# gabrieldemarmiesse/mojo-simdjson

Measured on AMD Instinct MI355X. Metric: stage-1 GB/s JSON ingested (+ % HBM3E peak), 1/2/4/8 MI355X, higher is better.
Workload: dtype u8

## Files before the change

### include/msj_stage1.h

```cpp
#ifndef MSJ_STAGE1_H
#define MSJ_STAGE1_H

#include <stdint.h>

#ifdef __cplusplus
extern "C" {
#endif

#define MSJ_SUCCESS 0
#define MSJ_CAPACITY 1
#define MSJ_MEMALLOC 2
#define MSJ_UTF8_ERROR 11
#define MSJ_EMPTY 13
#define MSJ_UNESCAPED_CHARS 14
#define MSJ_UNCLOSED_STRING 15
#define MSJ_UNEXPECTED_ERROR 24
#define MSJ_ERR_BAD_ARGUMENT (-1)
#define MSJ_ERR_NO_DEVICE (-2)
#define MSJ_ERR_HIP (-3)

#define MSJ_FLAG_STRICT_UTF8 1u
#define MSJ_FLAG_NO_UTF8 2u
#define MSJ_FLAG_TWO_PASS 0x100u
#define MSJ_FLAG_DEBUG_STALL 0x200u
// ... 112 lines not shown
int32_t msj_sharded_create(msj_ctx *ctx, const msj_exchange *xchg, const msj_sharded_ops *ops, msj_sharded **out);
void msj_sharded_destroy(msj_sharded *sh);
uint64_t msj_sharded_reruns(const msj_sharded *sh);
uint64_t msj_sharded_rounds(const msj_sharded *sh);
typedef struct msj_sharded_stats {
    uint64_t results, rounds, reruns;
    uint64_t stitch_device_ns, result_wait_ns;
    uint64_t kernel_device_ns;
    uint64_t last_kernel_ns;
    uint64_t last_stitch_ns;
    uint64_t reruns_behind_queue;
    uint64_t reserved[3];
} msj_sharded_stats;
int32_t msj_sharded_get_stats(const msj_sharded *sh, msj_sharded_stats *out);
#define MSJ_SHARDED_KERNEL_DONE 1
#define MSJ_SHARDED_REPORTS_IN 2
int32_t msj_sharded_ticket_state(msj_sharded *sh, uint32_t ticket);
void msj_exchange_release(msj_exchange *x);

int32_t msj_stage1_sharded_submit(msj_sharded *sh, const uint8_t *d_shard, uint64_t shard_len, uint32_t *d_idx,
                                  uint64_t idx_capacity, uint64_t total_len, int32_t has_prefix,
                                  const msj_carry *speculation, msj_segment *d_segments, uint32_t max_segments,
                                  void *stream, uint32_t flags, uint32_t *ticket_out);
typedef struct msj_shard_placement {
    uint64_t index_begin;
    uint64_t byte_base;
    uint64_t count;
    uint64_t bytes;
} msj_shard_placement;
int32_t msj_stage1_sharded_result(msj_sharded *sh, uint32_t ticket, int32_t *code_out, uint64_t *total_count_out,
                                  msj_carry *local_out, msj_carry *used_out, msj_shard_placement *placement_out);
int32_t msj_debug_set_pipeline_min_bytes(msj_ctx *ctx, uint64_t bytes);
int32_t msj_debug_fail_pipeline_setup(msj_ctx *ctx, int32_t on);
int32_t msj_debug_set_segment_bytes(msj_ctx *ctx, uint64_t bytes);

typedef struct msj_tokens_result {
    uint64_t n;
    int32_t final_depth;
    int32_t min_depth;
    int32_t max_depth;
    uint32_t reserved;
} msj_tokens_result;

int32_t msj_tokens_device(msj_ctx *ctx, const uint8_t *d_buf, uint64_t len, const uint32_t *d_idx, uint64_t n,
                          uint8_t *d_type, int32_t *d_depth, uint32_t *d_match, msj_tokens_result *d_result,
                          void *stream);
int32_t msj_tokens_chain_device(msj_ctx *ctx, const uint8_t *d_buf, uint64_t len, const uint32_t *d_idx, uint64_t n,
                                uint8_t *d_type, int32_t *d_depth, uint32_t *d_match, msj_tokens_result *d_result,
                                const msj_tokens_result *d_prev, void *stream);

#define MSJ_SPAN_STRING 1u
#define MSJ_SPAN_ESCAPED 2u
#define MSJ_SPAN_NUMBER 4u
#define MSJ_SPAN_FLOAT 8u
#define MSJ_SPAN_OPEN 16u
#define MSJ_SPAN_BAD 32u
#define MSJ_SPAN_LONG 128u
int32_t msj_token_spans_device(msj_ctx *ctx, const uint8_t *d_buf, uint64_t len, const uint32_t *d_idx, uint64_t n,
                               uint32_t *d_end, uint8_t *d_flags, void *stream);

typedef struct msj_bracket_pair {
    uint32_t open, close;
} msj_bracket_pair;
int32_t msj_tokens_pairs_device(msj_ctx *ctx, const uint8_t *d_buf, uint64_t len, const uint32_t *d_idx, uint64_t n, uint8_t *d_type,
                                int32_t *d_depth, msj_bracket_pair *d_pairs, msj_tokens_result *d_result,
                                const msj_tokens_result *d_prev, void *stream);
// ... 269 lines not shown
```

### mojo_simdjson_amd/csrc/ctx.h

```cpp
#pragma once
#include <hip/hip_runtime.h>

#include <mutex>
#include <vector>

#include "../../include/msj_stage1.h"
#include "launch.h"
#include "stage1_kernel.h"

#pragma GCC visibility push(hidden)

inline bool hip_ok(hipError_t e) { return e == hipSuccess; }
inline bool aligned(const void *p, uintptr_t a) { return (reinterpret_cast<uintptr_t>(p) & (a - 1)) == 0; }

struct DeviceBuffer {
    void *p = nullptr;
    uint64_t bytes = 0;
    DeviceBuffer() = default;
    DeviceBuffer(const DeviceBuffer &) = delete;
    DeviceBuffer &operator=(const DeviceBuffer &) = delete;
    ~DeviceBuffer() { release(); }
    bool reserve(uint64_t need, bool headroom) {
        if (need <= bytes) return true;
        release();
// ... 8 lines not shown
    void release() {
        if (p) {
            (void)hipDeviceSynchronize();
            (void)hipFree(p);
        }
        p = nullptr;
        bytes = 0;
    }
    template <class T>
    T *as() const { return static_cast<T *>(p); }
};

constexpr uint64_t kPipelineMinDefault = 64u << 20;

struct HostPipe;

struct msj_ctx {
    int device = 0;
    HostPipe *pipe = nullptr;
    DeviceBuffer ws;
    uint64_t ws_words = 0;
    uint32_t ws_toggle = 0;
    uint32_t ws_dirty[2] = {0, 0};
    msj_carry *carries = nullptr;
    uint32_t n_carries = 0;
    DeviceBuffer d_in, d_idx;
    msj_carry *d_result = nullptr;
    uint8_t *h_pin = nullptr;
    uint8_t *d_small = nullptr;
    uint32_t grid = 0;
    uint32_t wait_ticks = msj::kWaitTicksDefault;
    uint64_t seg_bytes = msj::kSegmentBytes;
    uint64_t pipeline_min = kPipelineMinDefault;
    bool pipe_unavailable = false;
    bool pipe_fail_setup = false;
    DeviceBuffer tp;
    uint64_t fallbacks = 0;
    struct {
        bool valid = false;
        const uint8_t *d_buf; uint64_t len; uint32_t *d_idx; uint64_t idx_capacity;
        const msj_carry *d_carry_in; msj_carry *d_carry_out; msj_segment *d_segments; uint32_t max_segments;
        bool has_prefix, is_final, no_emit; uint64_t trailer_len; hipStream_t stream; uint32_t flags;
        bool by_value; uint32_t carry_bits;
    } last;
    struct HostRange { const uint8_t *base; uint64_t bytes; };
    std::vector<HostRange> pinned;
    bool is_pinned(const void *p, uint64_t n) const {
        const uint8_t *q = static_cast<const uint8_t *>(p);
        for (const HostRange &r : pinned)
            if (q >= r.base && n <= r.bytes && (uint64_t)(q - r.base) <= r.bytes - n) return true;
        return false;
    }
    DeviceBuffer span_fix;
    DeviceBuffer tok_ws;
    uint64_t tok_doc_n = ~0ull;
    DeviceBuffer seg_idx;
    uint8_t *types_out = nullptr;
    DeviceBuffer resid;
    msj_token_opts tok_opts;
    DeviceBuffer doc_ws;
    DeviceBuffer num_ws;
    DeviceBuffer val_ws;
    DeviceBuffer vdoc_ws;
    DeviceBuffer tape_ws;
    DeviceBuffer tdoc_ws;
    DeviceBuffer sel_ws;
// ... 22 lines not shown
```

### mojo_simdjson_amd/csrc/host_pipe.cpp

```cpp
#include <atomic>
#include <chrono>
#include <condition_variable>
#include <cstdio>
#include <cstdlib>
#include <cstring>
#include <deque>
#include <functional>
#include <new>
#include <thread>

#include <pthread.h>
#include <sched.h>
#include <sys/syscall.h>
#include <unistd.h>

#include "ctx.h"

#pragma GCC visibility push(hidden)

struct GpuHostLocality {
    char pci[32] = "";
    int node = -1;
    cpu_set_t cpus;
    int n_cpus = 0;
    char link_speed[32] = "", link_width[16] = "";
};
static bool read_line(const char *path, char *out, size_t cap) {
    FILE *f = std::fopen(path, "r");
    if (!f) return false;
    const bool ok = std::fgets(out, (int)cap, f) != nullptr;
    std::fclose(f);
    if (ok) out[std::strcspn(out, "\n")] = 0;
    return ok;
}
static GpuHostLocality gpu_locality(int device) {
    GpuHostLocality g;
    CPU_ZERO(&g.cpus);
    char bus[32] = "";
    if (hipDeviceGetPCIBusId(bus, (int)sizeof bus, device) != hipSuccess) {
        (void)hipGetLastError();
        return g;
    }
    for (char *c = bus; *c; c++)
        if (*c >= 'A' && *c <= 'F') *c = (char)(*c - 'A' + 'a');
    std::snprintf(g.pci, sizeof g.pci, "%s", bus);
    char path[128], line[4096];
    std::snprintf(path, sizeof path, "/sys/bus/pci/devices/%s/numa_node", bus);
    if (read_line(path, line, sizeof line)) g.node = std::atoi(line);
    std::snprintf(path, sizeof path, "/sys/bus/pci/devices/%s/current_link_speed", bus);
    (void)read_line(path, g.link_speed, sizeof g.link_speed);
    std::snprintf(path, sizeof path, "/sys/bus/pci/devices/%s/current_link_width", bus);
    (void)read_line(path, g.link_width, sizeof g.link_width);
    std::snprintf(path, sizeof path, "/sys/bus/pci/devices/%s/local_cpulist", bus);
    cpu_set_t allowed;
    CPU_ZERO(&allowed);
    if (read_line(path, line, sizeof line) && sched_getaffinity(0, sizeof allowed, &allowed) == 0) {
        char *save = nullptr;
        for (char *tok = strtok_r(line, ",", &save); tok; tok = strtok_r(nullptr, ",", &save)) {
            int lo = 0, hi = 0;
            const int k = std::sscanf(tok, "%d-%d", &lo, &hi);
            if (k == 1) hi = lo;
            for (int c = lo; k >= 1 && c <= hi && c < CPU_SETSIZE; c++)
                if (CPU_ISSET(c, &allowed)) {
                    CPU_SET(c, &g.cpus);
                    g.n_cpus++;
                }
        }
    }
    return g;
}
static int numa_node_of(const void *p) {
#ifdef SYS_get_mempolicy
    int node = -1;
    if (p && syscall(SYS_get_mempolicy, &node, nullptr, 0UL, const_cast<void *>(p), 3UL ) == 0) return node;
#endif
    (void)p;
    return -1;
}

struct CopyPool {
    const cpu_set_t *bind = nullptr;
    int bound = 0;
    std::vector<std::thread> threads;
    std::deque<std::function<void()>> tasks;
    std::mutex m;
    std::condition_variable cv;
    bool stop = false;
    explicit CopyPool(int n, const cpu_set_t *cpus = nullptr) : bind(cpus) {
        std::atomic<int> ok{0};
        for (int i = 0; i < n; i++)
            threads.emplace_back([this, &ok] {
                if (bind && pthread_setaffinity_np(pthread_self(), sizeof(cpu_set_t), bind) == 0) ok.fetch_add(1);
                ok.fetch_add(1 << 16);
                for (;;) {
                    std::function<void()> f;
                    {
                        std::unique_lock<std::mutex> lk(m);
                        cv.wait(lk, [this] { return stop || !tasks.empty(); });
                        if (stop && tasks.empty()) return;
                        f = std::move(tasks.front());
                        tasks.pop_front();
                    }
                    f();
                }
            });
        while ((ok.load() >> 16) < n) std::this_thread::yield();
        bound = ok.load() & 0xFFFF;
    }
    ~CopyPool() {
        {
            std::lock_guard<std::mutex> lk(m);
            stop = true;
        }
        cv.notify_all();
        for (auto &t : threads) t.join();
    }
    void copy_async(void *dst, const void *src, uint64_t n, int parts, std::atomic<int> *pending) {
        if (parts < 1) parts = 1;
        pending->store(parts, std::memory_order_relaxed);
        const uint64_t step = ((n / parts) + 63) & ~63ull;
        for (int i = 0; i < parts; i++) {
            const uint64_t lo = step * i < n ? step * i : n, hi = (i + 1 == parts || step * (i + 1) > n) ? n : step * (i + 1);
            {
                std::lock_guard<std::mutex> lk(m);
                tasks.emplace_back([=] {
                    if (hi > lo) std::memcpy(static_cast<char *>(dst) + lo, static_cast<const char *>(src) + lo, hi - lo);
                    pending->fetch_sub(1, std::memory_order_release);
                });
            }
            cv.notify_one();
        }
    }
    static void wait(std::atomic<int> *pending) {
        while (pending->load(std::memory_order_acquire) != 0) std::this_thread::yield();
    }
    void copy(void *dst, const void *src, uint64_t n, int parts) {
        if (n < (1u << 20) || parts <= 1) {
            std::memcpy(dst, src, n);
            return;
        }
        std::mutex dm;
        std::condition_variable dcv;
        int left = parts;
        const uint64_t step = ((n / parts) + 63) & ~63ull;
        for (int i = 0; i < parts; i++) {
            const uint64_t lo = step * i < n ? step * i : n, hi = (i + 1 == parts || step * (i + 1) > n) ? n : step * (i + 1);
            {
                std::lock_guard<std::mutex> lk(m);
                tasks.emplace_back([=, &dm, &dcv, &left] {
                    if (hi > lo) std::memcpy(static_cast<char *>(dst) + lo, static_cast<const char *>(src) + lo, hi - lo);
                    std::lock_guard<std::mutex> g(dm);
                    if (--left == 0) dcv.notify_one();
                });
            }
            cv.notify_one();
        }
        std::unique_lock<std::mutex> lk(dm);
        dcv.wait(lk, [&] { return left == 0; });
    }
};

#ifdef MSJ_DEBUG_KNOBS
static int knob_int(const char *name, int dflt, int lo) {
    const char *v = std::getenv(name);
    const int x = v && *v ? std::atoi(v) : dflt;
    return x < lo ? lo : x;
}
bool knob_set(const char *name) { return std::getenv(name) != nullptr; }
#else
static int knob_int(const char *, int dflt, int) { return dflt; }
bool knob_set(const char *) { return false; }
#endif

struct HostPipe {
    static constexpr int kInSlots = 3, kOutSlots = 2;
    const int kCopyThreads = knob_int("MSJ_PIPE_THREADS", 8, 1), kParts = knob_int("MSJ_PIPE_PARTS", 4, 1);
    const bool direct_upload = knob_int("MSJ_PIPE_DIRECT_UPLOAD", 0, 0) != 0;
    static constexpr uint64_t kChunk = 16ull << 20;
    static constexpr uint64_t kPiece = 16ull << 20;
    uint8_t *pin_in[kInSlots] = {nullptr, nullptr, nullptr};
    uint8_t *pin_out[kOutSlots] = {nullptr, nullptr};
    msj_carry *h_carries = nullptr;
    msj_carry *d_carries = nullptr;
    uint64_t n_carries = 0;
    hipStream_t s_up = nullptr, s_k = nullptr, s_down = nullptr;
    hipEvent_t ev_in[kInSlots] = {nullptr, nullptr, nullptr};
    hipEvent_t ev_out[kOutSlots] = {nullptr, nullptr};
    std::vector<hipEvent_t> ev_chunk;
    GpuHostLocality where;
    CopyPool pool;
    bool ok = false;

    explicit HostPipe(int device) : where(gpu_locality(device)), pool(kCopyThreads, where.n_cpus > 0 ? &where.cpus : nullptr) {
        ok = true;
        std::thread([&] {
            (void)hipSetDevice(device);
            if (where.n_cpus > 0) (void)pthread_setaffinity_np(pthread_self(), sizeof(cpu_set_t), &where.cpus);
            for (auto &p : pin_in) {
                ok = ok && hip_ok(hipHostMalloc(reinterpret_cast<void **>(&p), kChunk, hipHostMallocDefault));
                if (ok) std::memset(p, 0, kChunk);
            }
            for (auto &p : pin_out) {
                ok = ok && hip_ok(hipHostMalloc(reinterpret_cast<void **>(&p), kPiece, hipHostMallocDefault));
                if (ok) std::memset(p, 0, kPiece);
            }
        }).join();
        ok = ok && hip_ok(hipStreamCreateWithFlags(&s_up, hipStreamNonBlocking)) &&
             hip_ok(hipStreamCreateWithFlags(&s_k, hipStreamNonBlocking)) &&
             hip_ok(hipStreamCreateWithFlags(&s_down, hipStreamNonBlocking));
        for (auto &e : ev_in) ok = ok && hip_ok(hipEventCreateWithFlags(&e, hipEventDisableTiming));
        for (auto &e : ev_out) ok = ok && hip_ok(hipEventCreateWithFlags(&e, hipEventDisableTiming));
    }
    ~HostPipe() {
        for (auto p : pin_in)
            if (p) (void)hipHostFree(p);
        for (auto p : pin_out)
            if (p) (void)hipHostFree(p);
        if (h_carries) (void)hipHostFree(h_carries);
        if (d_carries) (void)hipFree(d_carries);
        for (auto e : ev_in)
            if (e) (void)hipEventDestroy(e);
        for (auto e : ev_out)
            if (e) (void)hipEventDestroy(e);
        for (auto e : ev_chunk) (void)hipEventDestroy(e);
        if (s_up) (void)hipStreamDestroy(s_up);
        if (s_k) (void)hipStreamDestroy(s_k);
        if (s_down) (void)hipStreamDestroy(s_down);
    }
    bool reserve(uint64_t nchunks) {
        if (nchunks + 1 > n_carries) {
            if (h_carries) (void)hipHostFree(h_carries);
            if (d_carries) (void)hipFree(d_carries);
            h_carries = nullptr;
            d_carries = nullptr;
            n_carries = 0;
            if (!hip_ok(hipHostMalloc(reinterpret_cast<void **>(&h_carries), (nchunks + 1) * sizeof(msj_carry), hipHostMallocDefault)) ||
                !hip_ok(hipMalloc(reinterpret_cast<void **>(&d_carries), (nchunks + 1) * sizeof(msj_carry))))
                return false;
            n_carries = nchunks + 1;
        }
        while (ev_chunk.size() < nchunks) {
            hipEvent_t e;
            if (!hip_ok(hipEventCreateWithFlags(&e, hipEventDisableTiming))) return false;
            ev_chunk.push_back(e);
        }
        return true;
    }
};

void host_pipe_destroy(HostPipe *pipe) { delete pipe; }

int32_t host_pipeline(msj_ctx *ctx, const uint8_t *buf, uint64_t len, uint32_t *idx_out, uint64_t dev_cap, uint32_t flags,
                      msj_carry *res) {
    if (ctx->pipe_fail_setup) return kPipeUnavailable;
    if (!ctx->pipe) {
        ctx->pipe = new (std::nothrow) HostPipe(ctx->device);
        if (!ctx->pipe) return kPipeUnavailable;
    }
    HostPipe &P = *ctx->pipe;
    if (!P.ok) return kPipeUnavailable;
    uint8_t *const d_in = ctx->d_in.as<uint8_t>();
    uint32_t *const d_idx = ctx->d_idx.as<uint32_t>();
    const uint64_t chunk = HostPipe::kChunk;
    const uint64_t nchunks = (len + chunk - 1) / chunk;
    if (!P.reserve(nchunks)) return kPipeUnavailable;
    if (!hip_ok(hipMemsetAsync(&P.d_carries[0], 0, sizeof(msj_carry), P.s_k))) return kPipeUnavailable;

    static const bool trace = knob_set("MSJ_PIPE_TRACE");
    auto now = [] { return std::chrono::duration<double, std::milli>(std::chrono::steady_clock::now().time_since_epoch()).count(); };
    const double t_begin = now();
    std::vector<double> t_chunk_done(nchunks, 0.0), t_piece;
    const bool in_pinned = P.direct_upload || ctx->is_pinned(buf, len);
    const bool out_pinned = ctx->is_pinned(idx_out, dev_cap * sizeof(uint32_t));
    int32_t down_rc = MSJ_SUCCESS;
    std::atomic<bool> abort{false};
    std::atomic<uint64_t> recorded{0};
    std::thread down([&] {
        (void)hipSetDevice(ctx->device);
        uint64_t sent = 0, pieces = 0;
        std::atomic<int> copying[HostPipe::kOutSlots];
        for (auto &c : copying) c.store(0);
        for (uint64_t k = 0; k < nchunks; k++) {
            while (recorded.load(std::memory_order_acquire) <= k && !abort.load()) std::this_thread::yield();
            if (abort.load()) break;
            if (!hip_ok(hipEventSynchronize(P.ev_chunk[k]))) { down_rc = MSJ_ERR_HIP; break; }
            if (abort.load()) break;
            if (trace) t_chunk_done[k] = now() - t_begin;
            const msj_carry &c = P.h_carries[k + 1];
            const bool last = k + 1 == nchunks;
            uint64_t avail = c.count;
            if (last && (c.code == MSJ_SUCCESS || c.code == MSJ_EMPTY || c.code == MSJ_UTF8_ERROR)) avail += 3;
            if (avail > dev_cap) avail = dev_cap;
            if (out_pinned) {
                if (avail > sent &&
                    !hip_ok(hipMemcpyAsync(idx_out + sent, d_idx + sent, (avail - sent) * sizeof(uint32_t), hipMemcpyDeviceToHost, P.s_down))) {
                    down_rc = MSJ_ERR_HIP;
                    break;
                }
                sent = avail;
                if (trace) t_piece.push_back(now() - t_begin);
                continue;
            }
            const uint64_t piece = HostPipe::kPiece / sizeof(uint32_t);
            while (sent < avail) {
                const uint64_t mis = sent & 63u;
                const uint64_t n = avail - sent < piece - mis ? avail - sent : piece - mis;
                const int slot = (int)(pieces % HostPipe::kOutSlots);
                CopyPool::wait(&copying[slot]);
                if (!hip_ok(hipMemcpyAsync(P.pin_out[slot], d_idx + (sent - mis), (n + mis) * sizeof(uint32_t), hipMemcpyDeviceToHost, P.s_down)) ||
                    !hip_ok(hipStreamSynchronize(P.s_down))) {
                    down_rc = MSJ_ERR_HIP;
                    break;
                }
                P.pool.copy_async(idx_out + sent, P.pin_out[slot] + mis * sizeof(uint32_t), n * sizeof(uint32_t), P.kParts, &copying[slot]);
                sent += n;
                pieces++;
                if (trace) t_piece.push_back(now() - t_begin);
            }
            if (down_rc != MSJ_SUCCESS) break;
        }
        for (auto &c : copying) CopyPool::wait(&c);
        if (out_pinned && !hip_ok(hipStreamSynchronize(P.s_down))) down_rc = MSJ_ERR_HIP;
    });

    double t_copy = 0, t_wait = 0;
    int32_t rc = MSJ_SUCCESS;
    for (uint64_t k = 0; k < nchunks && rc == MSJ_SUCCESS; k++) {
        const uint64_t off = k * chunk, n = len - off < chunk ? len - off : chunk;
        const int slot = (int)(k % HostPipe::kInSlots);
        double t0 = now();
        if (in_pinned) {
            if (!hip_ok(hipMemcpyAsync(d_in + off, buf + off, n, hipMemcpyHostToDevice, P.s_up))) rc = MSJ_ERR_HIP;
            t_copy += now() - t0;
        } else {
            if (k >= (uint64_t)HostPipe::kInSlots && !hip_ok(hipEventSynchronize(P.ev_in[slot]))) rc = MSJ_ERR_HIP;
            double t1 = now();
            if (rc == MSJ_SUCCESS) P.pool.copy(P.pin_in[slot], buf + off, n, P.kParts);
            t_wait += t1 - t0;
            t_copy += now() - t1;
            if (rc == MSJ_SUCCESS && !hip_ok(hipMemcpyAsync(d_in + off, P.pin_in[slot], n, hipMemcpyHostToDevice, P.s_up)))
                rc = MSJ_ERR_HIP;
        }
        if (rc == MSJ_SUCCESS && (!hip_ok(hipEventRecord(P.ev_in[slot], P.s_up)) || !hip_ok(hipStreamWaitEvent(P.s_k, P.ev_in[slot], 0))))
            rc = MSJ_ERR_HIP;
        if (rc == MSJ_SUCCESS)
            rc = enqueue_shard(ctx, d_in + off, n, d_idx, dev_cap, &P.d_carries[k], &P.d_carries[k + 1], nullptr, 0, nullptr,
                               k > 0, k + 1 == nchunks, false, len, P.s_k, flags, (uint32_t)off);
        if (rc == MSJ_SUCCESS &&
            (!hip_ok(hipMemcpyAsync(&P.h_carries[k + 1], &P.d_carries[k + 1], sizeof(msj_carry), hipMemcpyDeviceToHost, P.s_k)) ||
             !hip_ok(hipEventRecord(P.ev_chunk[k], P.s_k))))
            rc = MSJ_ERR_HIP;
        if (rc == MSJ_SUCCESS) recorded.store(k + 1, std::memory_order_release);
        if (rc != MSJ_SUCCESS) {
            abort.store(true);
            for (uint64_t j = k; j < nchunks; j++) (void)hipEventRecord(P.ev_chunk[j], P.s_k);
        }
    }
    const double t_up = now();
    down.join();
    (void)hipStreamSynchronize(P.s_k);
    if (trace)
        std::fprintf(stderr, "msj host pipeline: %llu chunks, upload loop %.2f ms (slot waits %.2f, staging copies %.2f), "
                             "then %.2f ms until the last index was down\n",
                     (unsigned long long)nchunks, t_up - t_begin, t_wait, t_copy, now() - t_up);
    if (trace) {
        std::fprintf(stderr, "  chunk results seen at (ms):");
        for (double t : t_chunk_done) std::fprintf(stderr, " %.2f", t);
        std::fprintf(stderr, "\n  download pieces issued+previous copied out at (ms):");
        for (double t : t_piece) std::fprintf(stderr, " %.2f", t);
        std::fprintf(stderr, "\n");
    }
    ctx->last.valid = false;
    if (rc != MSJ_SUCCESS) return rc;
    if (down_rc != MSJ_SUCCESS) return down_rc;
    *res = P.h_carries[nchunks];
    return MSJ_SUCCESS;
}
#pragma GCC visibility pop

extern "C" {

int32_t msj_host_placement(msj_ctx *ctx, char *out, uint64_t capacity) {
    if (!out || capacity == 0) return MSJ_ERR_BAD_ARGUMENT;
    std::unique_lock<std::mutex> lock(g_default_mutex, std::defer_lock);
    if (!ctx) {
        lock.lock();
        ctx = default_ctx_locked();
        if (!ctx) return MSJ_ERR_NO_DEVICE;
    }
    const GpuHostLocality g = ctx->pipe ? ctx->pipe->where : gpu_locality(ctx->device);
    const int ring_in = ctx->pipe ? numa_node_of(ctx->pipe->pin_in[0]) : -1, ring_out = ctx->pipe ? numa_node_of(ctx->pipe->pin_out[0]) : -1;
    int nodes = 0;
    for (;; nodes++) {
        char path[64];
        std::snprintf(path, sizeof path, "/sys/devices/system/node/node%d", nodes);
        if (access(path, F_OK) != 0) break;
    }
    const int n = std::snprintf(out, (size_t)capacity,
                                "{\"gpu_pci\": \"%s\", \"gpu_numa_node\": %d, \"numa_nodes\": %d, \"gpu_local_cpus_usable\": %d, "
                                "\"pipeline_created\": %s, \"copy_threads\": %d, \"copy_threads_bound_to_gpu_node\": %d, "
                                "\"ring_in_node\": %d, \"ring_out_node\": %d, \"pcie_link_speed\": \"%s\", \"pcie_link_width\": \"%s\"}",
                                g.pci, g.node, nodes, g.n_cpus, ctx->pipe ? "true" : "false", ctx->pipe ? ctx->pipe->kCopyThreads : 0,
                                ctx->pipe ? ctx->pipe->pool.bound : 0, ring_in, ring_out, g.link_speed, g.link_width);
    return (n < 0 || (uint64_t)n >= capacity) ? MSJ_CAPACITY : MSJ_SUCCESS;
}

int32_t msj_debug_numa_node_of(const void *host_ptr) { return numa_node_of(host_ptr); }

}
```

Measured before the change: 3441.

## Restructure host pipeline into slot-ring issuer/drainer with L3-spread copy workers

Replaces the host staging pipeline with explicit input/output slot rings (4 in, 3 out by default instead of 3/2), a templated issuer and drainer state machine, a persistent parked drainer thread, and a lock-light ring-based copy pool whose workers are spread across L3 cache domains of the GPU-local CPUs. Chunks come from a schedule helper that can cap the chunk size. The aim is to overlap host staging copies, H2D uploads, kernels and D2H downloads more deeply, and to cut per-call thread creation and std::function queue overhead. In exchange it adds more pinned memory, more complex synchronisation, and affinity choices that depend on sysfs topology.

```diff
diff --git a/include/msj_stage1.h b/include/msj_stage1.h
--- a/include/msj_stage1.h
+++ b/include/msj_stage1.h
@@ -168,6 +168,7 @@
                                   msj_carry *local_out, msj_carry *used_out, msj_shard_placement *placement_out);
 int32_t msj_debug_set_pipeline_min_bytes(msj_ctx *ctx, uint64_t bytes);
 int32_t msj_debug_fail_pipeline_setup(msj_ctx *ctx, int32_t on);
+int32_t msj_debug_set_pipeline_chunk_bytes(msj_ctx *ctx, uint64_t bytes);
 int32_t msj_debug_set_segment_bytes(msj_ctx *ctx, uint64_t bytes);
 
 typedef struct msj_tokens_result {
diff --git a/mojo_simdjson_amd/csrc/ctx.h b/mojo_simdjson_amd/csrc/ctx.h
--- a/mojo_simdjson_amd/csrc/ctx.h
+++ b/mojo_simdjson_amd/csrc/ctx.h
@@ -64,6 +64,7 @@
     uint32_t wait_ticks = msj::kWaitTicksDefault;
     uint64_t seg_bytes = msj::kSegmentBytes;
     uint64_t pipeline_min = kPipelineMinDefault;
+    uint64_t pipe_chunk_max = 0;
     bool pipe_unavailable = false;
     bool pipe_fail_setup = false;
     DeviceBuffer tp;
diff --git a/mojo_simdjson_amd/csrc/host_pipe.cpp b/mojo_simdjson_amd/csrc/host_pipe.cpp
--- a/mojo_simdjson_amd/csrc/host_pipe.cpp
+++ b/mojo_simdjson_amd/csrc/host_pipe.cpp
@@ -4,8 +4,6 @@
 #include <cstdio>
 #include <cstdlib>
 #include <cstring>
-#include <deque>
-#include <functional>
 #include <new>
 #include <thread>
 
@@ -15,6 +13,8 @@
 #include <unistd.h>
 
 #include "ctx.h"
+#include "pipe_schedule.h"
+#include "pipe_slots.h"
 
 #pragma GCC visibility push(hidden)
 
@@ -69,6 +69,50 @@
     }
     return g;
 }
+struct WorkerCpus {
+    static constexpr int kMaxSets = 32;
+    cpu_set_t sets[kMaxSets];
+    int n = 0;
+    int domains = 0;
+};
+static void parse_cpulist(char *line, cpu_set_t *out) {
+    CPU_ZERO(out);
+    char *save = nullptr;
+    for (char *tok = strtok_r(line, ",", &save); tok; tok = strtok_r(nullptr, ",", &save)) {
+        int lo = 0, hi = 0;
+        const int k = std::sscanf(tok, "%d-%d", &lo, &hi);
+        if (k == 1) hi = lo;
+        for (int c = lo; k >= 1 && c <= hi && c < CPU_SETSIZE; c++) CPU_SET(c, out);
+    }
+}
+static void worker_cpus(const GpuHostLocality &g, int workers, WorkerCpus *w) {
+    cpu_set_t domains[WorkerCpus::kMaxSets], seen;
+    int nd = 0;
+    CPU_ZERO(&seen);
+    for (int c = 0; c < CPU_SETSIZE && nd < WorkerCpus::kMaxSets; c++) {
+        if (!CPU_ISSET(c, &g.cpus) || CPU_ISSET(c, &seen)) continue;
+        char path[128], line[4096];
+        cpu_set_t l3;
+        std::snprintf(path, sizeof path, "/sys/devices/system/cpu/cpu%d/cache/index3/shared_cpu_list", c);
+        if (!read_line(path, line, sizeof line)) {
+            nd = 0;
+            break;
+        }
+        parse_cpulist(line, &l3);
+        CPU_SET(c, &l3);
+        CPU_AND(&domains[nd], &l3, &g.cpus);
+        CPU_OR(&seen, &seen, &l3);
+        nd++;
+    }
+    w->domains = nd;
+    if (nd <= 1) {
+        w->sets[0] = g.cpus;
+        w->n = 1;
+        return;
+    }
+    w->n = nd < workers ? nd : workers;
+    for (int i = 0; i < w->n; i++) w->sets[i] = domains[(int)((long)i * nd / w->n)];
+}
 static int numa_node_of(const void *p) {
 #ifdef SYS_get_mempolicy
     int node = -1;
@@ -78,138 +122,75 @@
     return -1;
 }
 
-struct CopyPool {
-    const cpu_set_t *bind = nullptr;
-    int bound = 0;
-    std::vector<std::thread> threads;
-    std::deque<std::function<void()>> tasks;
-    std::mutex m;
-    std::condition_variable cv;
-    bool stop = false;
-    explicit CopyPool(int n, const cpu_set_t *cpus = nullptr) : bind(cpus) {
-        std::atomic<int> ok{0};
-        for (int i = 0; i < n; i++)
-            threads.emplace_back([this, &ok] {
-                if (bind && pthread_setaffinity_np(pthread_self(), sizeof(cpu_set_t), bind) == 0) ok.fetch_add(1);
-                ok.fetch_add(1 << 16);
-                for (;;) {
-                    std::function<void()> f;
-                    {
-                        std::unique_lock<std::mutex> lk(m);
-                        cv.wait(lk, [this] { return stop || !tasks.empty(); });
-                        if (stop && tasks.empty()) return;
-                        f = std::move(tasks.front());
-                        tasks.pop_front();
-                    }
-                    f();
-                }
-            });
-        while ((ok.load() >> 16) < n) std::this_thread::yield();
-        bound = ok.load() & 0xFFFF;
-    }
-    ~CopyPool() {
-        {
-            std::lock_guard<std::mutex> lk(m);
-            stop = true;
-        }
-        cv.notify_all();
-        for (auto &t : threads) t.join();
-    }
-    void copy_async(void *dst, const void *src, uint64_t n, int parts, std::atomic<int> *pending) {
-        if (parts < 1) parts = 1;
-        pending->store(parts, std::memory_order_relaxed);
-        const uint64_t step = ((n / parts) + 63) & ~63ull;
-        for (int i = 0; i < parts; i++) {
-            const uint64_t lo = step * i < n ? step * i : n, hi = (i + 1 == parts || step * (i + 1) > n) ? n : step * (i + 1);
-            {
-                std::lock_guard<std::mutex> lk(m);
-                tasks.emplace_back([=] {
-                    if (hi > lo) std::memcpy(static_cast<char *>(dst) + lo, static_cast<const char *>(src) + lo, hi - lo);
-                    pending->fetch_sub(1, std::memory_order_release);
-                });
-            }
-            cv.notify_one();
-        }
-    }
-    static void wait(std::atomic<int> *pending) {
-        while (pending->load(std::memory_order_acquire) != 0) std::this_thread::yield();
-    }
-    void copy(void *dst, const void *src, uint64_t n, int parts) {
-        if (n < (1u << 20) || parts <= 1) {
-            std::memcpy(dst, src, n);
-            return;
-        }
-        std::mutex dm;
-        std::condition_variable dcv;
-        int left = parts;
-        const uint64_t step = ((n / parts) + 63) & ~63ull;
-        for (int i = 0; i < parts; i++) {
-            const uint64_t lo = step * i < n ? step * i : n, hi = (i + 1 == parts || step * (i + 1) > n) ? n : step * (i + 1);
-            {
-                std::lock_guard<std::mutex> lk(m);
-                tasks.emplace_back([=, &dm, &dcv, &left] {
-                    if (hi > lo) std::memcpy(static_cast<char *>(dst) + lo, static_cast<const char *>(src) + lo, hi - lo);
-                    std::lock_guard<std::mutex> g(dm);
-                    if (--left == 0) dcv.notify_one();
-                });
-            }
-            cv.notify_one();
-        }
-        std::unique_lock<std::mutex> lk(dm);
-        dcv.wait(lk, [&] { return left == 0; });
-    }
-};
-
 #ifdef MSJ_DEBUG_KNOBS
-static int knob_int(const char *name, int dflt, int lo) {
+static int knob_int(const char *name, int dflt, int lo, int hi = 1 << 20) {
     const char *v = std::getenv(name);
     const int x = v && *v ? std::atoi(v) : dflt;
-    return x < lo ? lo : x;
+    return x < lo ? lo : x > hi ? hi : x;
 }
 bool knob_set(const char *name) { return std::getenv(name) != nullptr; }
 #else
-static int knob_int(const char *, int dflt, int) { return dflt; }
+static int knob_int(const char *, int dflt, int, int = 0) { return dflt; }
 bool knob_set(const char *) { return false; }
 #endif
 
 struct HostPipe {
-    static constexpr int kInSlots = 3, kOutSlots = 2;
+    static constexpr int kMaxIn = msj_pipe::kMaxSlots, kMaxOut = msj_pipe::kMaxSlots;
+    const int kInSlots = knob_int("MSJ_PIPE_IN_SLOTS", 4, 2, kMaxIn), kOutSlots = knob_int("MSJ_PIPE_OUT_SLOTS", 3, 2, kMaxOut);
     const int kCopyThreads = knob_int("MSJ_PIPE_THREADS", 8, 1), kParts = knob_int("MSJ_PIPE_PARTS", 4, 1);
     const bool direct_upload = knob_int("MSJ_PIPE_DIRECT_UPLOAD", 0, 0) != 0;
     static constexpr uint64_t kChunk = 16ull << 20;
     static constexpr uint64_t kPiece = 16ull << 20;
-    uint8_t *pin_in[kInSlots] = {nullptr, nullptr, nullptr};
-    uint8_t *pin_out[kOutSlots] = {nullptr, nullptr};
+    uint8_t *pin_in[kMaxIn] = {};
+    uint8_t *pin_out[kMaxOut] = {};
     msj_carry *h_carries = nullptr;
     msj_carry *d_carries = nullptr;
     uint64_t n_carries = 0;
     hipStream_t s_up = nullptr, s_k = nullptr, s_down = nullptr;
-    hipEvent_t ev_in[kInSlots] = {nullptr, nullptr, nullptr};
-    hipEvent_t ev_out[kOutSlots] = {nullptr, nullptr};
+    hipEvent_t ev_in[kMaxIn] = {};
+    hipEvent_t ev_out[kMaxOut] = {};
     std::vector<hipEvent_t> ev_chunk;
+    std::vector<msj_pipe::Chunk> chunks;
     GpuHostLocality where;
-    CopyPool pool;
+    const bool bind_workers;
+    WorkerCpus worker_sets;
+    msj_pipe::CopyPool pool;
+    int device;
+    msj_pipe::ParkedThread drainer;
     bool ok = false;
 
-    explicit HostPipe(int device) : where(gpu_locality(device)), pool(kCopyThreads, where.n_cpus > 0 ? &where.cpus : nullptr) {
+    WorkerCpus deal_workers() const {
+        WorkerCpus w;
+        if (knob_int("MSJ_PIPE_SPREAD", 1, 0) != 0) {
+            worker_cpus(where, kCopyThreads, &w);
+        } else {
+            w.sets[0] = where.cpus;
+            w.n = 1;
+        }
+        return w;
+    }
+    explicit HostPipe(int dev)
+        : where(gpu_locality(dev)), bind_workers(where.n_cpus >= kCopyThreads), worker_sets(deal_workers()),
+          pool(kCopyThreads, worker_sets.sets, bind_workers ? worker_sets.n : 0),
+          device(dev), drainer([](void *p) { (void)hipSetDevice(static_cast<HostPipe *>(p)->device); }, this) {
         ok = true;
         std::thread([&] {
             (void)hipSetDevice(device);
             if (where.n_cpus > 0) (void)pthread_setaffinity_np(pthread_self(), sizeof(cpu_set_t), &where.cpus);
-            for (auto &p : pin_in) {
-                ok = ok && hip_ok(hipHostMalloc(reinterpret_cast<void **>(&p), kChunk, hipHostMallocDefault));
-                if (ok) std::memset(p, 0, kChunk);
+            for (int i = 0; i < kInSlots; i++) {
+                ok = ok && hip_ok(hipHostMalloc(reinterpret_cast<void **>(&pin_in[i]), kChunk, hipHostMallocDefault));
+                if (ok) std::memset(pin_in[i], 0, kChunk);
             }
-            for (auto &p : pin_out) {
-                ok = ok && hip_ok(hipHostMalloc(reinterpret_cast<void **>(&p), kPiece, hipHostMallocDefault));
-                if (ok) std::memset(p, 0, kPiece);
+            for (int i = 0; i < kOutSlots; i++) {
+                ok = ok && hip_ok(hipHostMalloc(reinterpret_cast<void **>(&pin_out[i]), kPiece, hipHostMallocDefault));
+                if (ok) std::memset(pin_out[i], 0, kPiece);
             }
         }).join();
         ok = ok && hip_ok(hipStreamCreateWithFlags(&s_up, hipStreamNonBlocking)) &&
              hip_ok(hipStreamCreateWithFlags(&s_k, hipStreamNonBlocking)) &&
              hip_ok(hipStreamCreateWithFlags(&s_down, hipStreamNonBlocking));
-        for (auto &e : ev_in) ok = ok && hip_ok(hipEventCreateWithFlags(&e, hipEventDisableTiming));
-        for (auto &e : ev_out) ok = ok && hip_ok(hipEventCreateWithFlags(&e, hipEventDisableTiming));
+        for (int i = 0; i < kInSlots; i++) ok = ok && hip_ok(hipEventCreateWithFlags(&ev_in[i], hipEventDisableTiming));
+        for (int i = 0; i < kOutSlots; i++) ok = ok && hip_ok(hipEventCreateWithFlags(&ev_out[i], hipEventDisableTiming));
     }
     ~HostPipe() {
         for (auto p : pin_in)
@@ -250,6 +231,96 @@
 
 void host_pipe_destroy(HostPipe *pipe) { delete pipe; }
 
+static int event_state(hipEvent_t e) {
+    const hipError_t r = hipEventQuery(e);
+    if (r == hipSuccess) return 1;
+    (void)hipGetLastError();
+    return r == hipErrorNotReady ? 0 : -1;
+}
+
+struct PipeCall {
+    static constexpr int kQueryError = MSJ_ERR_HIP;
+    msj_ctx *ctx;
+    HostPipe &P;
+    const uint8_t *buf;
+    uint64_t len;
+    uint32_t *idx_out;
+    uint64_t dev_cap;
+    uint32_t flags;
+    uint8_t *d_in;
+    uint32_t *d_idx;
+    bool in_pinned, out_pinned;
+    uint64_t piece_words;
+    msj_pipe::PipeShared shared;
+    msj_pipe::OutRing out;
+    int32_t down_rc = MSJ_SUCCESS;
+    bool trace = false;
+    double t_begin = 0;
+    std::vector<double> t_chunk_done, t_piece;
+    int drainer_cpu = -1;
+
+    static double now() { return std::chrono::duration<double, std::milli>(std::chrono::steady_clock::now().time_since_epoch()).count(); }
+
+    void stage(uint64_t k, int slot, std::atomic<int> *pending) {
+        if (in_pinned) pending->store(0, std::memory_order_relaxed);
+        else P.pool.copy_async(P.pin_in[slot], buf + P.chunks[k].offset, P.chunks[k].bytes, P.kParts, pending);
+    }
+    int issue(uint64_t k, int slot) {
+        const uint64_t off = P.chunks[k].offset, n = P.chunks[k].bytes, nchunks = P.chunks.size();
+        const uint8_t *src = in_pinned ? buf + off : P.pin_in[slot];
+        if (!hip_ok(hipMemcpyAsync(d_in + off, src, n, hipMemcpyHostToDevice, P.s_up)) || !hip_ok(hipEventRecord(P.ev_in[slot], P.s_up)) ||
+            !hip_ok(hipStreamWaitEvent(P.s_k, P.ev_in[slot], 0)))
+            return MSJ_ERR_HIP;
+        const int32_t rc = enqueue_shard(ctx, d_in + off, n, d_idx, dev_cap, &P.d_carries[k], &P.d_carries[k + 1], nullptr, 0, nullptr, k > 0,
+                                         k + 1 == nchunks, false, len, P.s_k, flags, (uint32_t)off);
+        if (rc != MSJ_SUCCESS) return rc;
+        if (!hip_ok(hipMemcpyAsync(&P.h_carries[k + 1], &P.d_carries[k + 1], sizeof(msj_carry), hipMemcpyDeviceToHost, P.s_k)) ||
+            !hip_ok(hipEventRecord(P.ev_chunk[k], P.s_k)))
+            return MSJ_ERR_HIP;
+        return MSJ_SUCCESS;
+    }
+    int h2d_done(int slot) { return in_pinned ? 1 : event_state(P.ev_in[slot]); }
+    void quiesce_up() {
+        (void)hipStreamSynchronize(P.s_up);
+        (void)hipStreamSynchronize(P.s_k);
+    }
+
+    int chunk_done(uint64_t k) {
+        const int s = event_state(P.ev_chunk[k]);
+        if (s == 1 && trace) t_chunk_done[k] = now() - t_begin;
+        return s;
+    }
+    uint64_t chunk_avail(uint64_t k) const {
+        const msj_carry &c = P.h_carries[k + 1];
+        uint64_t avail = c.count;
+        if (k + 1 == P.chunks.size() && (c.code == MSJ_SUCCESS || c.code == MSJ_EMPTY || c.code == MSJ_UTF8_ERROR)) avail += 3;
+        return avail > dev_cap ? dev_cap : avail;
+    }
+    int d2h(int slot, uint64_t sent, uint64_t words, uint64_t mis) {
+        if (trace) t_piece.push_back(now() - t_begin);
+        return hip_ok(hipMemcpyAsync(P.pin_out[slot], d_idx + (sent - mis), (words + mis) * sizeof(uint32_t), hipMemcpyDeviceToHost, P.s_down)) &&
+                       hip_ok(hipEventRecord(P.ev_out[slot], P.s_down))
+                   ? MSJ_SUCCESS
+                   : MSJ_ERR_HIP;
+    }
+    int d2h_done(int slot) { return event_state(P.ev_out[slot]); }
+    void copy_out(int slot, uint64_t sent, uint64_t words, uint64_t mis, std::atomic<int> *pending) {
+        P.pool.copy_async(idx_out + sent, P.pin_out[slot] + mis * sizeof(uint32_t), words * sizeof(uint32_t), P.kParts, pending);
+    }
+    bool direct() const { return out_pinned; }
+    int d2h_direct(uint64_t sent, uint64_t words) {
+        if (trace) t_piece.push_back(now() - t_begin);
+        return hip_ok(hipMemcpyAsync(idx_out + sent, d_idx + sent, words * sizeof(uint32_t), hipMemcpyDeviceToHost, P.s_down)) ? MSJ_SUCCESS : MSJ_ERR_HIP;
+    }
+    int quiesce_down() { return hip_ok(hipStreamSynchronize(P.s_down)) ? MSJ_SUCCESS : MSJ_ERR_HIP; }
+
+    static void drain(void *self) {
+        PipeCall &c = *static_cast<PipeCall *>(self);
+        if (c.trace) c.drainer_cpu = sched_getcpu();
+        c.down_rc = msj_pipe::run_drainer(c, c.out, c.P.chunks.size(), c.piece_words, &c.shared);
+    }
+};
+
 int32_t host_pipeline(msj_ctx *ctx, const uint8_t *buf, uint64_t len, uint32_t *idx_out, uint64_t dev_cap, uint32_t flags,
                       msj_carry *res) {
     if (ctx->pipe_fail_setup) return kPipeUnavailable;
@@ -259,120 +330,42 @@
     }
     HostPipe &P = *ctx->pipe;
     if (!P.ok) return kPipeUnavailable;
-    uint8_t *const d_in = ctx->d_in.as<uint8_t>();
-    uint32_t *const d_idx = ctx->d_idx.as<uint32_t>();
-    const uint64_t chunk = HostPipe::kChunk;
-    const uint64_t nchunks = (len + chunk - 1) / chunk;
+    static const uint64_t dflt_chunk = (uint64_t)knob_int("MSJ_PIPE_CHUNK_MIB", (int)(HostPipe::kChunk >> 20), 1, (int)(HostPipe::kChunk >> 20)) << 20;
+    const uint64_t max_chunk = ctx->pipe_chunk_max && ctx->pipe_chunk_max < HostPipe::kChunk ? ctx->pipe_chunk_max : dflt_chunk;
+    msj_pipe::chunk_schedule(len, max_chunk, &P.chunks);
+    const uint64_t nchunks = P.chunks.size();
     if (!P.reserve(nchunks)) return kPipeUnavailable;
     if (!hip_ok(hipMemsetAsync(&P.d_carries[0], 0, sizeof(msj_carry), P.s_k))) return kPipeUnavailable;
 
     static const bool trace = knob_set("MSJ_PIPE_TRACE");
-    auto now = [] { return std::chrono::duration<double, std::milli>(std::chrono::steady_clock::now().time_since_epoch()).count(); };
-    const double t_begin = now();
-    std::vector<double> t_chunk_done(nchunks, 0.0), t_piece;
-    const bool in_pinned = P.direct_upload || ctx->is_pinned(buf, len);
-    const bool out_pinned = ctx->is_pinned(idx_out, dev_cap * sizeof(uint32_t));
-    int32_t down_rc = MSJ_SUCCESS;
-    std::atomic<bool> abort{false};
-    std::atomic<uint64_t> recorded{0};
-    std::thread down([&] {
-        (void)hipSetDevice(ctx->device);
-        uint64_t sent = 0, pieces = 0;
-        std::atomic<int> copying[HostPipe::kOutSlots];
-        for (auto &c : copying) c.store(0);
-        for (uint64_t k = 0; k < nchunks; k++) {
-            while (recorded.load(std::memory_order_acquire) <= k && !abort.load()) std::this_thread::yield();
-            if (abort.load()) break;
-            if (!hip_ok(hipEventSynchronize(P.ev_chunk[k]))) { down_rc = MSJ_ERR_HIP; break; }
-            if (abort.load()) break;
-            if (trace) t_chunk_done[k] = now() - t_begin;
-            const msj_carry &c = P.h_carries[k + 1];
-            const bool last = k + 1 == nchunks;
-            uint64_t avail = c.count;
-            if (last && (c.code == MSJ_SUCCESS || c.code == MSJ_EMPTY || c.code == MSJ_UTF8_ERROR)) avail += 3;
-            if (avail > dev_cap) avail = dev_cap;
-            if (out_pinned) {
-                if (avail > sent &&
-                    !hip_ok(hipMemcpyAsync(idx_out + sent, d_idx + sent, (avail - sent) * sizeof(uint32_t), hipMemcpyDeviceToHost, P.s_down))) {
-                    down_rc = MSJ_ERR_HIP;
-                    break;
-                }
-                sent = avail;
-                if (trace) t_piece.push_back(now() - t_begin);
-                continue;
-            }
-            const uint64_t piece = HostPipe::kPiece / sizeof(uint32_t);
-            while (sent < avail) {
-                const uint64_t mis = sent & 63u;
-                const uint64_t n = avail - sent < piece - mis ? avail - sent : piece - mis;
-                const int slot = (int)(pieces % HostPipe::kOutSlots);
-                CopyPool::wait(&copying[slot]);
-                if (!hip_ok(hipMemcpyAsync(P.pin_out[slot], d_idx + (sent - mis), (n + mis) * sizeof(uint32_t), hipMemcpyDeviceToHost, P.s_down)) ||
-                    !hip_ok(hipStreamSynchronize(P.s_down))) {
-                    down_rc = MSJ_ERR_HIP;
-                    break;
-                }
-                P.pool.copy_async(idx_out + sent, P.pin_out[slot] + mis * sizeof(uint32_t), n * sizeof(uint32_t), P.kParts, &copying[slot]);
-                sent += n;
-                pieces++;
-                if (trace) t_piece.push_back(now() - t_begin);
-            }
-            if (down_rc != MSJ_SUCCESS) break;
-        }
-        for (auto &c : copying) CopyPool::wait(&c);
-        if (out_pinned && !hip_ok(hipStreamSynchronize(P.s_down))) down_rc = MSJ_ERR_HIP;
-    });
-
-    double t_copy = 0, t_wait = 0;
-    int32_t rc = MSJ_SUCCESS;
-    for (uint64_t k = 0; k < nchunks && rc == MSJ_SUCCESS; k++) {
-        const uint64_t off = k * chunk, n = len - off < chunk ? len - off : chunk;
-        const int slot = (int)(k % HostPipe::kInSlots);
-        double t0 = now();
-        if (in_pinned) {
-            if (!hip_ok(hipMemcpyAsync(d_in + off, buf + off, n, hipMemcpyHostToDevice, P.s_up))) rc = MSJ_ERR_HIP;
-            t_copy += now() - t0;
-        } else {
-            if (k >= (uint64_t)HostPipe::kInSlots && !hip_ok(hipEventSynchronize(P.ev_in[slot]))) rc = MSJ_ERR_HIP;
-            double t1 = now();
-            if (rc == MSJ_SUCCESS) P.pool.copy(P.pin_in[slot], buf + off, n, P.kParts);
-            t_wait += t1 - t0;
-            t_copy += now() - t1;
-            if (rc == MSJ_SUCCESS && !hip_ok(hipMemcpyAsync(d_in + off, P.pin_in[slot], n, hipMemcpyHostToDevice, P.s_up)))
-                rc = MSJ_ERR_HIP;
-        }
-        if (rc == MSJ_SUCCESS && (!hip_ok(hipEventRecord(P.ev_in[slot], P.s_up)) || !hip_ok(hipStreamWaitEvent(P.s_k, P.ev_in[slot], 0))))
-            rc = MSJ_ERR_HIP;
-        if (rc == MSJ_SUCCESS)
-            rc = enqueue_shard(ctx, d_in + off, n, d_idx, dev_cap, &P.d_carries[k], &P.d_carries[k + 1], nullptr, 0, nullptr,
-                               k > 0, k + 1 == nchunks, false, len, P.s_k, flags, (uint32_t)off);
-        if (rc == MSJ_SUCCESS &&
-            (!hip_ok(hipMemcpyAsync(&P.h_carries[k + 1], &P.d_carries[k + 1], sizeof(msj_carry), hipMemcpyDeviceToHost, P.s_k)) ||
-             !hip_ok(hipEventRecord(P.ev_chunk[k], P.s_k))))
-            rc = MSJ_ERR_HIP;
-        if (rc == MSJ_SUCCESS) recorded.store(k + 1, std::memory_order_release);
-        if (rc != MSJ_SUCCESS) {
-            abort.store(true);
-            for (uint64_t j = k; j < nchunks; j++) (void)hipEventRecord(P.ev_chunk[j], P.s_k);
-        }
-    }
-    const double t_up = now();
-    down.join();
+    PipeCall call{ctx, P, buf, len, idx_out, dev_cap, flags, ctx->d_in.as<uint8_t>(), ctx->d_idx.as<uint32_t>(),
+                  P.direct_upload || ctx->is_pinned(buf, len), ctx->is_pinned(idx_out, dev_cap * sizeof(uint32_t)),
+                  (max_chunk < HostPipe::kPiece ? max_chunk : HostPipe::kPiece) / sizeof(uint32_t), {}, msj_pipe::OutRing(P.kOutSlots)};
+    call.trace = trace;
+    call.t_begin = PipeCall::now();
+    const int cpu_begin = trace ? sched_getcpu() : -1;
+    if (trace) call.t_chunk_done.assign(nchunks, 0.0);
+    P.drainer.start(&PipeCall::drain, &call);
+    msj_pipe::InRing in(P.kInSlots);
+    msj_pipe::IssuerTimes times;
+    const int32_t rc = msj_pipe::run_issuer(call, in, nchunks, &call.shared, trace ? &times : nullptr);
+    const double t_up = PipeCall::now();
+    P.drainer.wait();
     (void)hipStreamSynchronize(P.s_k);
-    if (trace)
-        std::fprintf(stderr, "msj host pipeline: %llu chunks, upload loop %.2f ms (slot waits %.2f, staging copies %.2f), "
+    if (trace) {
+        std::fprintf(stderr, "msj host pipeline: %llu chunks, upload loop %.2f ms (slot waits %.2f, waits for staging copies %.2f), "
                              "then %.2f ms until the last index was down\n",
-                     (unsigned long long)nchunks, t_up - t_begin, t_wait, t_copy, now() - t_up);
-    if (trace) {
+                     (unsigned long long)nchunks, t_up - call.t_begin, times.wait_slot, times.wait_stage, PipeCall::now() - t_up);
+        std::fprintf(stderr, "  issuer on cpu %d -> %d, drainer on cpu %d\n", cpu_begin, sched_getcpu(), call.drainer_cpu);
         std::fprintf(stderr, "  chunk results seen at (ms):");
-        for (double t : t_chunk_done) std::fprintf(stderr, " %.2f", t);
-        std::fprintf(stderr, "\n  download pieces issued+previous copied out at (ms):");
-        for (double t : t_piece) std::fprintf(stderr, " %.2f", t);
+        for (double t : call.t_chunk_done) std::fprintf(stderr, " %.2f", t);
+        std::fprintf(stderr, "\n  download pieces issued at (ms):");
+        for (double t : call.t_piece) std::fprintf(stderr, " %.2f", t);
         std::fprintf(stderr, "\n");
     }
     ctx->last.valid = false;
     if (rc != MSJ_SUCCESS) return rc;
-    if (down_rc != MSJ_SUCCESS) return down_rc;
+    if (call.down_rc != MSJ_SUCCESS) return call.down_rc;
     *res = P.h_carries[nchunks];
     return MSJ_SUCCESS;
 }
@@ -399,12 +392,27 @@
     const int n = std::snprintf(out, (size_t)capacity,
                                 "{\"gpu_pci\": \"%s\", \"gpu_numa_node\": %d, \"numa_nodes\": %d, \"gpu_local_cpus_usable\": %d, "
                                 "\"pipeline_created\": %s, \"copy_threads\": %d, \"copy_threads_bound_to_gpu_node\": %d, "
-                                "\"ring_in_node\": %d, \"ring_out_node\": %d, \"pcie_link_speed\": \"%s\", \"pcie_link_width\": \"%s\"}",
+                                "\"ring_in_node\": %d, \"ring_out_node\": %d, \"pcie_link_speed\": \"%s\", \"pcie_link_width\": \"%s\", "
+                                "\"copy_threads_bind_wanted\": %s, \"gpu_node_l3_domains\": %d, \"copy_thread_cpu_sets\": %d}",
                                 g.pci, g.node, nodes, g.n_cpus, ctx->pipe ? "true" : "false", ctx->pipe ? ctx->pipe->kCopyThreads : 0,
-                                ctx->pipe ? ctx->pipe->pool.bound : 0, ring_in, ring_out, g.link_speed, g.link_width);
+                                ctx->pipe ? ctx->pipe->pool.bound : 0, ring_in, ring_out, g.link_speed, g.link_width,
+                                ctx->pipe ? (ctx->pipe->bind_workers ? "true" : "false") : "null",
+                                ctx->pipe ? ctx->pipe->worker_sets.domains : -1, ctx->pipe && ctx->pipe->bind_workers ? ctx->pipe->worker_sets.n : 0);
     return (n < 0 || (uint64_t)n >= capacity) ? MSJ_CAPACITY : MSJ_SUCCESS;
 }
 
+int32_t msj_debug_set_pipeline_chunk_bytes(msj_ctx *ctx, uint64_t bytes) {
+    if (bytes % msj_pipe::kScheduleTile != 0 || bytes > HostPipe::kChunk) return MSJ_ERR_BAD_ARGUMENT;
+    std::unique_lock<std::mutex> lock(g_default_mutex, std::defer_lock);
+    if (!ctx) {
+        lock.lock();
+        ctx = default_ctx_locked();
+        if (!ctx) return MSJ_ERR_NO_DEVICE;
+    }
+    ctx->pipe_chunk_max = bytes;
+    return MSJ_SUCCESS;
+}
+
 int32_t msj_debug_numa_node_of(const void *host_ptr) { return numa_node_of(host_ptr); }
 
 }
diff --git a/mojo_simdjson_amd/csrc/pipe_schedule.h b/mojo_simdjson_amd/csrc/pipe_schedule.h
--- /dev/null
+++ b/mojo_simdjson_amd/csrc/pipe_schedule.h
@@ -0,0 +1,47 @@
+#pragma once
+#include <cstdint>
+#include <vector>
+
+namespace msj_pipe {
+
+constexpr uint64_t kScheduleTile = 4096;
+constexpr uint64_t kRampDivisor = 8;
+
+struct Chunk {
+    uint64_t offset, bytes;
+};
+
+constexpr uint64_t kScheduleSlack = 10;
+
+inline void chunk_schedule(uint64_t len, uint64_t max_chunk, std::vector<Chunk> *out) {
+    out->clear();
+    if (len == 0) return;
+    const uint64_t max_t = max_chunk / kScheduleTile ? max_chunk / kScheduleTile : 1;
+    const uint64_t min_t = max_t / kRampDivisor ? max_t / kRampDivisor : 1;
+    const uint64_t tiles = (len + kScheduleTile - 1) / kScheduleTile;
+    std::vector<uint64_t> head, tail;
+    uint64_t lo = 0, hi = tiles, step = min_t;
+    while (step < max_t && hi - lo > 2 * step) {
+        head.push_back(step);
+        tail.push_back(step);
+        lo += step;
+        hi -= step;
+        step = 2 * step < max_t ? 2 * step : max_t;
+    }
+    const uint64_t mid = hi - lo, nmid = (mid + max_t - 1) / max_t;
+    uint64_t at = 0;
+    auto emit = [&](uint64_t t) {
+        const uint64_t off = at * kScheduleTile, end = (at + t) * kScheduleTile < len ? (at + t) * kScheduleTile : len;
+        out->push_back({off, end - off});
+        at += t;
+    };
+    for (uint64_t t : head) emit(t);
+    for (uint64_t i = 0, left = mid; i < nmid; i++) {
+        const uint64_t t = (left + (nmid - i) - 1) / (nmid - i);
+        emit(t);
+        left -= t;
+    }
+    for (size_t i = tail.size(); i-- > 0;) emit(tail[i]);
+}
+
+}
diff --git a/mojo_simdjson_amd/csrc/pipe_slots.h b/mojo_simdjson_amd/csrc/pipe_slots.h
--- /dev/null
+++ b/mojo_simdjson_amd/csrc/pipe_slots.h
@@ -0,0 +1,316 @@
+#pragma once
+#include <atomic>
+#include <condition_variable>
+#include <cstdint>
+#include <cstring>
+#include <mutex>
+#include <thread>
+#include <vector>
+
+#include <pthread.h>
+#include <sched.h>
+
+namespace msj_pipe {
+
+struct CopyPool {
+    struct Slice {
+        void *dst;
+        const void *src;
+        uint64_t n;
+        std::atomic<int> *pending;
+    };
+    static constexpr uint32_t kQueue = 256;
+    int bound = 0;
+    std::vector<std::thread> threads;
+    Slice ring[kQueue];
+    uint32_t head = 0, tail = 0;
+    std::mutex m;
+    std::condition_variable cv, cv_room;
+    bool stop = false;
+
+    explicit CopyPool(int n, const cpu_set_t *sets = nullptr, int nsets = 0) {
+        std::atomic<int> ok{0};
+        for (int i = 0; i < n; i++)
+            threads.emplace_back([this, sets, nsets, i, &ok] {
+                if (nsets > 0 && pthread_setaffinity_np(pthread_self(), sizeof(cpu_set_t), &sets[i % nsets]) == 0) ok.fetch_add(1);
+                ok.fetch_add(1 << 16);
+                work();
+            });
+        while ((ok.load() >> 16) < n) std::this_thread::yield();
+        bound = ok.load() & 0xFFFF;
+    }
+    ~CopyPool() {
+        {
+            std::lock_guard<std::mutex> lk(m);
+            stop = true;
+        }
+        cv.notify_all();
+        for (auto &t : threads) t.join();
+    }
+    void work() {
+        for (;;) {
+            Slice s;
+            {
+                std::unique_lock<std::mutex> lk(m);
+                cv.wait(lk, [this] { return stop || head != tail; });
+                if (head == tail) return;
+                s = ring[head % kQueue];
+                head++;
+            }
+            cv_room.notify_one();
+            if (s.n) std::memcpy(s.dst, s.src, s.n);
+            s.pending->fetch_sub(1, std::memory_order_release);
+        }
+    }
+    void copy_async(void *dst, const void *src, uint64_t n, int parts, std::atomic<int> *pending) {
+        if (parts < 1) parts = 1;
+        if ((uint32_t)parts > kQueue / 2) parts = (int)(kQueue / 2);
+        if (n < (uint64_t)parts * 65536) parts = (int)(n / 65536) ? (int)(n / 65536) : 1;
+        pending->store(parts, std::memory_order_relaxed);
+        const uint64_t step = ((n / parts) + 63) & ~63ull;
+        {
+            std::unique_lock<std::mutex> lk(m);
+            cv_room.wait(lk, [&] { return tail - head + (uint32_t)parts <= kQueue; });
+            for (int i = 0; i < parts; i++) {
+                const uint64_t lo = step * i < n ? step * i : n, hi = (i + 1 == parts || step * (i + 1) > n) ? n : step * (i + 1);
+                ring[tail % kQueue] = Slice{static_cast<char *>(dst) + lo, static_cast<const char *>(src) + lo, hi - lo, pending};
+                tail++;
+            }
+        }
+        if (parts == 1) cv.notify_one();
+        else cv.notify_all();
+    }
+    static void wait(const std::atomic<int> *pending) {
+        while (pending->load(std::memory_order_acquire) != 0) std::this_thread::yield();
+    }
+};
+
+class ParkedThread {
+    std::mutex m;
+    std::condition_variable cv;
+    void (*fn)(void *) = nullptr;
+    void *arg = nullptr;
+    bool busy = false, stop = false;
+    std::thread t;
+
+public:
+    explicit ParkedThread(void (*init)(void *) = nullptr, void *init_arg = nullptr) {
+        t = std::thread([this, init, init_arg] {
+            if (init) init(init_arg);
+            std::unique_lock<std::mutex> lk(m);
+            for (;;) {
+                cv.wait(lk, [this] { return stop || (busy && fn); });
+                if (stop) return;
+                void (*f)(void *) = fn;
+                void *a = arg;
+                lk.unlock();
+                f(a);
+                lk.lock();
+                fn = nullptr;
+                busy = false;
+                cv.notify_all();
+            }
+        });
+    }
+    ~ParkedThread() {
+        {
+            std::unique_lock<std::mutex> lk(m);
+            cv.wait(lk, [this] { return !busy; });
+            stop = true;
+        }
+        cv.notify_all();
+        t.join();
+    }
+    void start(void (*f)(void *), void *a) {
+        {
+            std::lock_guard<std::mutex> lk(m);
+            fn = f;
+            arg = a;
+            busy = true;
+        }
+        cv.notify_all();
+    }
+    void wait() {
+        std::unique_lock<std::mutex> lk(m);
+        cv.wait(lk, [this] { return !busy; });
+    }
+};
+
+struct PipeShared {
+    std::atomic<uint64_t> recorded{0};
+    std::atomic<bool> abort{false};
+};
+
+enum class InState : uint8_t { Free, Staging, Staged, InFlight };
+enum class OutState : uint8_t { Free, InFlight, Landed };
+
+constexpr int kMaxSlots = 8;
+
+struct InRing {
+    int slots;
+    InState state[kMaxSlots];
+    std::atomic<int> pending[kMaxSlots];
+    explicit InRing(int n) : slots(n) {
+        for (int i = 0; i < kMaxSlots; i++) {
+            state[i] = InState::Free;
+            pending[i].store(0);
+        }
+    }
+    bool all_free() const {
+        for (int i = 0; i < slots; i++)
+            if (state[i] != InState::Free || pending[i].load() != 0) return false;
+        return true;
+    }
+};
+struct OutRing {
+    int slots;
+    OutState state[kMaxSlots];
+    std::atomic<int> pending[kMaxSlots];
+    uint64_t sent[kMaxSlots], words[kMaxSlots], mis[kMaxSlots];
+    explicit OutRing(int n) : slots(n) {
+        for (int i = 0; i < kMaxSlots; i++) {
+            state[i] = OutState::Free;
+            pending[i].store(0);
+            sent[i] = words[i] = mis[i] = 0;
+        }
+    }
+    bool all_free() const {
+        for (int i = 0; i < slots; i++)
+            if (state[i] != OutState::Free || pending[i].load() != 0) return false;
+        return true;
+    }
+};
+
+struct IssuerTimes {
+    double wait_slot = 0, wait_stage = 0;
+};
+
+template <class Backend>
+int run_issuer(Backend &b, InRing &ring, uint64_t nchunks, PipeShared *shared, IssuerTimes *times = nullptr) {
+    uint64_t submitted = 0, issued = 0, freed = 0;
+    int rc = 0;
+    bool peer_failed = false;
+    while (issued < nchunks && rc == 0) {
+        if (shared->abort.load(std::memory_order_acquire)) {
+            peer_failed = true;
+            break;
+        }
+        bool progress = false;
+        while (freed < issued) {
+            const int slot = (int)(freed % ring.slots), done = b.h2d_done(slot);
+            if (done < 0) rc = Backend::kQueryError;
+            if (done <= 0) break;
+            ring.state[slot] = InState::Free;
+            freed++;
+            progress = true;
+        }
+        if (rc != 0) break;
+        while (submitted < nchunks && submitted - freed < (uint64_t)ring.slots) {
+            const int slot = (int)(submitted % ring.slots);
+            ring.state[slot] = InState::Staging;
+            b.stage(submitted, slot, &ring.pending[slot]);
+            submitted++;
+            progress = true;
+        }
+        if (issued < submitted) {
+            const int slot = (int)(issued % ring.slots);
+            if (ring.pending[slot].load(std::memory_order_acquire) == 0) {
+                ring.state[slot] = InState::Staged;
+                rc = b.issue(issued, slot);
+                if (rc != 0) break;
+                ring.state[slot] = InState::InFlight;
+                issued++;
+                shared->recorded.store(issued, std::memory_order_release);
+                continue;
+            }
+        }
+        if (!progress) {
+            const double t0 = times ? b.now() : 0;
+            std::this_thread::yield();
+            if (times) (issued == submitted ? times->wait_slot : times->wait_stage) += b.now() - t0;
+        }
+    }
+    if (rc != 0 || peer_failed) {
+        shared->abort.store(true, std::memory_order_release);
+        for (int i = 0; i < ring.slots; i++) CopyPool::wait(&ring.pending[i]);
+        b.quiesce_up();
+    }
+    for (int i = 0; i < ring.slots; i++) ring.state[i] = InState::Free;
+    return rc;
+}
+
+template <class Backend>
+int run_drainer(Backend &b, OutRing &ring, uint64_t nchunks, uint64_t piece_words, PipeShared *shared) {
+    uint64_t k = 0, avail = 0, sent = 0;
+    uint64_t issued = 0, landed = 0, freed = 0;
+    int rc = 0;
+    bool peer_failed = false;
+    const bool direct = b.direct();
+    for (;;) {
+        if (shared->abort.load(std::memory_order_acquire)) {
+            peer_failed = true;
+            break;
+        }
+        bool progress = false;
+        while (freed < landed && ring.pending[freed % ring.slots].load(std::memory_order_acquire) == 0) {
+            ring.state[freed % ring.slots] = OutState::Free;
+            freed++;
+            progress = true;
+        }
+        while (k < nchunks && shared->recorded.load(std::memory_order_acquire) > k) {
+            const int done = b.chunk_done(k);
+            if (done < 0) rc = Backend::kQueryError;
+            if (done <= 0) break;
+            avail = b.chunk_avail(k);
+            k++;
+            progress = true;
+        }
+        if (rc != 0) break;
+        if (direct) {
+            if (sent < avail) {
+                rc = b.d2h_direct(sent, avail - sent);
+                if (rc != 0) break;
+                sent = avail;
+                progress = true;
+            }
+        } else {
+            while (sent < avail && issued - freed < (uint64_t)ring.slots) {
+                const int slot = (int)(issued % ring.slots);
+                const uint64_t mis = sent & 63u;
+                const uint64_t n = avail - sent < piece_words - mis ? avail - sent : piece_words - mis;
+                rc = b.d2h(slot, sent, n, mis);
+                if (rc != 0) break;
+                ring.state[slot] = OutState::InFlight;
+                ring.sent[slot] = sent;
+                ring.words[slot] = n;
+                ring.mis[slot] = mis;
+                sent += n;
+                issued++;
+                progress = true;
+            }
+            if (rc != 0) break;
+            while (landed < issued) {
+                const int slot = (int)(landed % ring.slots), done = b.d2h_done(slot);
+                if (done < 0) rc = Backend::kQueryError;
+                if (done <= 0) break;
+                ring.state[slot] = OutState::Landed;
+                b.copy_out(slot, ring.sent[slot], ring.words[slot], ring.mis[slot], &ring.pending[slot]);
+                landed++;
+                progress = true;
+            }
+            if (rc != 0) break;
+        }
+        if (k == nchunks && sent == avail && freed == issued) break;
+        if (!progress) std::this_thread::yield();
+    }
+    if (rc != 0) shared->abort.store(true, std::memory_order_release);
+    if (rc != 0 || peer_failed || direct) {
+        for (int i = 0; i < ring.slots; i++) CopyPool::wait(&ring.pending[i]);
+        const int q = b.quiesce_down();
+        if (rc == 0) rc = q;
+    }
+    for (int i = 0; i < ring.slots; i++) ring.state[i] = OutState::Free;
+    return rc;
+}
+
+}
```

Result: no change. 3442 (median of 2 runs) (+0.0%).
